# ajgupta93/d4pg-pytorch

Hardware: NVIDIA H100
Metric: learner grad-steps/sec (batch 256, 51 atoms) (higher is better)
Workload: dtype f32

## Files before the change

d4pg-pytorch_b200/csrc/learner.cu:

```cuda
#include "common.cuh"
#include "gemm_ffma.cuh"
#include "adam.cuh"
#include <string.h>
#include <stdlib.h>
#include <initializer_list>
#include <new>
#include <string>
#include <vector>

#include "internal.cuh"
#include "mlp_chain.cuh"
#include "mlp_tc_chain.cuh"

namespace d4pg {

struct Batch { float *s, *a, *s2; double* r; uint8_t* done; int32_t* idx; float* wts; uint8_t* hz; };

struct Workspace {
  Batch batch[2];
  float *h1[5], *h2[5], *h3[5], *out[5];
  float *m, *q_probs, *target_probs, *dlogits_q, *dlogits_pi, *loss_rows, *pi_rows;
  float *c_dz22, *c_dz2, *c_dz1, *p_dz22, *p_dz2, *a_dz3, *a_dz22, *a_dh2, *a_dz1;
  LearnerClock* clock;
  float* xchg;
  unsigned long long* pipe_epoch;
  double* sq_partials;
  int64_t total;
};

enum StepPlan { PLAN_LEVELS, PLAN_CHAIN, PLAN_TC_CHAIN };
constexpr int CHAIN_MAX_BATCH = 512;
static bool chain_pre_ok(const d4pg_learner_config_t& c) { return c.precision == 0 && c.act_dim <= 8; }
static bool chain_plan_fits(const d4pg_learner_config_t& c) {
  const int H = D4PG_HIDDEN, S = c.obs_dim, A = c.act_dim, N = c.n_atoms;
  ChainArgs f, b;
  chain_args_begin(f, c.batch, nullptr, c.precision);
  chain_add(f, 0, chain_fwd(nullptr, 0, nullptr, H, S, EPI_BIAS_RELU, nullptr, 0, 1));
  chain_add(f, 0, chain_fwd(nullptr, 0, nullptr, H, H, EPI_BIAS_RELU, nullptr, 0, 1));
  ChainSlot fc2 = chain_fwd(nullptr, 0, nullptr, H, H + A, EPI_BIAS_RELU, nullptr, 0, 1);
  if (chain_pre_ok(c)) chain_pre_layer(fc2, nullptr, 0, nullptr, nullptr, 0, A, H, EPI_BIAS_TANH, nullptr, 0, 0, H, false);
  else chain_add(f, 0, chain_fwd(nullptr, 0, nullptr, A, H, EPI_BIAS_TANH, nullptr, 0, 1));
  chain_add(f, 0, fc2);
  chain_add(f, 0, chain_fwd(nullptr, 0, nullptr, N, H, EPI_BIAS, nullptr, 0, 0));
  chain_args_begin(b, c.batch, nullptr, c.precision);
  chain_add(b, 0, chain_dx(nullptr, 0, H, N, EPI_RELU_MASK, nullptr, 0, nullptr, 0, 1));
  chain_add(b, 0, chain_dx(nullptr, 0, H, H, EPI_RELU_MASK, nullptr, 0, nullptr, 0, 1));
  ChainSlot fc3 = chain_dx(nullptr, 0, H, A, EPI_RELU_MASK, nullptr, 0, nullptr, 0, 1);
// ... 21 lines not shown
  auto take = [&](int64_t n) { float* p = base ? base + off : nullptr; off += align4(n); return p; };
  const int H = D4PG_HIDDEN, Sp = pitch4(S), Ap = pitch4(A), Np = pitch4(N);
  auto take_rows = [&](Batch& h) {
    h.s = take(int64_t(B) * Sp); h.a = take(int64_t(B) * Ap); h.s2 = take(int64_t(B) * Sp);
    h.r = reinterpret_cast<double*>(take(int64_t(B) * 2));
    h.done = reinterpret_cast<uint8_t*>(take((B + 3) / 4));
  };
  take_rows(w.batch[0]);
  for (int k = 0; k < 5; ++k) {
    if (k != 4) w.h1[k] = take(int64_t(B) * H);
    w.h2[k] = take(int64_t(B) * H); w.h3[k] = take(int64_t(B) * H);
  }
  w.out[0] = take(int64_t(B) * Ap); w.out[3] = take(int64_t(B) * Ap);
  w.out[1] = take(int64_t(B) * Np); w.out[2] = take(int64_t(B) * Np); w.out[4] = take(int64_t(B) * Np);
  w.m = take(int64_t(B) * Np); w.q_probs = take(int64_t(B) * Np); w.target_probs = take(int64_t(B) * Np);
  w.dlogits_q = take(int64_t(B) * Np); w.dlogits_pi = take(int64_t(B) * Np);
  w.loss_rows = take(B); w.pi_rows = take(B);
  w.c_dz22 = take(int64_t(B) * H); w.c_dz2 = take(int64_t(B) * H); w.c_dz1 = take(int64_t(B) * H);
  w.p_dz22 = take(int64_t(B) * H); w.p_dz2 = take(int64_t(B) * H);
  w.a_dz3 = take(int64_t(B) * Ap); w.a_dz22 = take(int64_t(B) * H); w.a_dh2 = take(int64_t(B) * H);
  w.a_dz1 = take(int64_t(B) * H);
  w.clock = reinterpret_cast<LearnerClock*>(take(sizeof(LearnerClock) / 4 + 4));
  w.xchg = plan != PLAN_LEVELS ? take(std::max(chain_xchg_floats(B), tcc_xchg_floats(B))) : nullptr;
  w.pipe_epoch = reinterpret_cast<unsigned long long*>(take(2 * int64_t((B + SAMPLE_ROWS - 1) / SAMPLE_ROWS)));
  if (prefetch) {
    take_rows(w.batch[1]);
    for (int k = 0; k < 2; ++k) { w.batch[k].idx = reinterpret_cast<int32_t*>(take(B)); w.batch[k].wts = take(B); }
  }
  if (clip) w.sq_partials = reinterpret_cast<double*>(take(2 * GRAD_NORM_CTAS * 2));
  if (tails)
    for (int k = 0; k < (prefetch ? 2 : 1); ++k) w.batch[k].hz = reinterpret_cast<uint8_t*>(take((B + 3) / 4));
  w.total = off;
  return w;
}
}

using namespace d4pg;

struct d4pg_learner {
  d4pg_learner_config_t cfg;
  d4pg_learner_buffers_t buf;
  d4pg_replay* replay;
  d4pg_comm* comm;
  StepPlan plan;
  Workspace ws;
  NetDims da, dc;
// ... 136 lines not shown
}
#define RUN(name, repeatable, call) \
  do { if (int rc_ = run_launch(x, name, repeatable, [&] { return (call); })) return rc_; } while (0)
static int run_level(Step& x, std::initializer_list<GemmProblem> problems) {
  GemmBatch g;
  gemm_batch_begin(g);
  for (const GemmProblem& p : problems) gemm_batch_add(g, p);
  RUN("gemm_launch", !gemm_batch_has_splitk(g), gemm_launch(g, x.c.precision, x.st));
  return D4PG_OK;
}

static int sample_batch(Step& x) {
  const d4pg_learner_config_t& c = x.c;
  RUN("learner_sample", false,
      learner_sample(x.L->replay, x.B, c.prioritized, c.sample_mode == 0 ? x.b.uniforms : nullptr,
                     (c.sample_mode == 0 && !c.prioritized) ? x.b.positions : nullptr,
                     c.philox_seed, x.w.clock, x.L->clock_params,
                     x.bt.idx, x.bt.wts, x.bt.s, x.bt.a, x.bt.r, x.bt.s2, x.bt.done, x.bt.hz, x.Sp, x.Ap, x.L->norm_affine,
                     x.L->norm_clip, x.pf ? x.par : -1, x.st));
  return D4PG_OK;
}

static void tcc_begin(const Step& x, TccArgs& a, int step_slot) {
  tcc_args_begin(a, x.B, reinterpret_cast<uint8_t*>(x.w.xchg), x.c.precision == 1 ? 3 : 1);
  a.step_slot = step_slot;
}
static int tcc_fwd_group(TccArgs& fa, int ci, int sl, const Step& x, Net net, int l, float* C, int ldc, int publish) {
  const Layer y = layer(x.L, net, l);
  return tcc_slot_group(fa, ci, sl, x.L->tcc_img[fwd_image(net, l)], y.epi, y.bias, nullptr, 0, C, ldc, publish);
}
static void tcc_build_actor_critic(TccArgs& fa, int ci, const Step& x, Net an, Net cn, const float* s, int ka, int kc,
                                   bool keep, bool actor_only = false) {
  const Workspace& w = x.w;
  const int H = D4PG_HIDDEN;
  int l, p1, p2 = -1;
  tcc_chain_x0(fa, ci, s, x.Sp, x.S);
  l = tcc_slot_begin(fa, ci); tcc_slot_src_x(fa, ci, l);
  p1 = tcc_fwd_group(fa, ci, l, x, an, 0, keep ? w.h1[ka] : nullptr, H, 1);
  if (!actor_only) p2 = tcc_fwd_group(fa, ci, l, x, cn, 0, nullptr, H, 1);
  l = tcc_slot_begin(fa, ci); tcc_slot_src_plane(fa, ci, l, p1, 8);
  p1 = tcc_fwd_group(fa, ci, l, x, an, 1, keep ? w.h2[ka] : nullptr, H, 1);
  l = tcc_slot_begin(fa, ci); tcc_slot_src_plane(fa, ci, l, p1, 8);
  p1 = tcc_fwd_group(fa, ci, l, x, an, 2, keep ? w.h3[ka] : nullptr, H, 1);
  l = tcc_slot_begin(fa, ci); tcc_slot_src_plane(fa, ci, l, p1, 8);
  const int pa = tcc_fwd_group(fa, ci, l, x, an, 3, w.out[ka], x.Ap, 1);
  if (actor_only) return;
  l = tcc_slot_begin(fa, ci); tcc_slot_src_plane(fa, ci, l, p2, 8); tcc_slot_src_plane(fa, ci, l, pa, 1);
// ... 551 lines not shown
    const size_t nb = size_t(cfg->batch);
    bool ok = cudaEventCreateWithFlags(&L->ev_in, cudaEventDisableTiming) == cudaSuccess &&
              cudaEventCreateWithFlags(&L->ev_out, cudaEventDisableTiming) == cudaSuccess &&
              cudaHostAlloc(reinterpret_cast<void**>(&L->host_losses), 4 * sizeof(float), cudaHostAllocDefault) == cudaSuccess;
    for (int i = 0; i < 2 && ok; ++i)
      ok = cudaEventCreateWithFlags(&L->ev_loss[i], cudaEventDisableTiming) == cudaSuccess &&
           cudaHostAlloc(reinterpret_cast<void**>(&L->loss_ring[i]), 4 * sizeof(float), cudaHostAllocDefault) == cudaSuccess;
    for (int i = 0; i < 4 && ok; ++i)
      ok = cudaEventCreateWithFlags(&L->ev_h2d[i], cudaEventDisableTiming) == cudaSuccess &&
           cudaHostAlloc(reinterpret_cast<void**>(&L->host_u[i]), nb * sizeof(double), cudaHostAllocMapped) == cudaSuccess &&
           cudaHostAlloc(reinterpret_cast<void**>(&L->host_pos[i]), nb * sizeof(int32_t), cudaHostAllocMapped) == cudaSuccess;
    if (!ok) { set_error("d4pg_learner_create: pinned staging allocation failed"); delete L; return D4PG_ECUDA; }
  }
  if (cudaStreamCreateWithFlags(&L->side, cudaStreamNonBlocking) != cudaSuccess ||
      cudaEventCreateWithFlags(&L->ev_fork, cudaEventDisableTiming) != cudaSuccess ||
      cudaEventCreateWithFlags(&L->ev_join, cudaEventDisableTiming) != cudaSuccess ||
      cudaEventCreateWithFlags(&L->ev_fork2, cudaEventDisableTiming) != cudaSuccess ||
      cudaEventCreateWithFlags(&L->ev_join2, cudaEventDisableTiming) != cudaSuccess) {
    set_error("d4pg_learner_create: stream/event creation failed"); delete L; return D4PG_ECUDA;
  }
  trace_set_side_stream(L->side);
  cudaError_t e = cudaMemset(L->ws.clock, 0, sizeof(LearnerClock));
  if (e == cudaSuccess) e = cudaMemset(L->ws.pipe_epoch, 0, sizeof(unsigned long long) * size_t(cdiv(cfg->batch, SAMPLE_ROWS)));
  if (e != cudaSuccess) { set_error("d4pg_learner_create: %s", cudaGetErrorString(e)); delete L; return D4PG_ECUDA; }
  *out = L;
  return D4PG_OK;
}

extern "C" int32_t d4pg_learner_destroy(d4pg_learner_t* L) {
  if (!L) return D4PG_OK;
  for (int i = 0; i < 4; ++i) if (L->graph_exec[i]) cudaGraphExecDestroy(L->graph_exec[i]);
  for (int i = 0; i < 2; ++i) if (L->multi_exec[i]) cudaGraphExecDestroy(L->multi_exec[i]);
  cudaEventDestroy(L->ev_fork); cudaEventDestroy(L->ev_join); cudaEventDestroy(L->ev_fork2); cudaEventDestroy(L->ev_join2);
  cudaStreamDestroy(L->side);
  if (L->tcc_images) cudaFree(L->tcc_images);
  if (L->gtab) cudaFree(L->gtab);
  if (L->ing) { cudaStreamSynchronize(L->ing); cudaStreamDestroy(L->ing); }
  if (L->ev_ing) cudaEventDestroy(L->ev_ing);
  if (L->ev_in) cudaEventDestroy(L->ev_in);
  if (L->ev_out) cudaEventDestroy(L->ev_out);
  if (L->host_losses) cudaFreeHost(L->host_losses);
  for (int i = 0; i < 2; ++i) {
    if (L->ev_loss[i]) cudaEventDestroy(L->ev_loss[i]);
    if (L->loss_ring[i]) cudaFreeHost(L->loss_ring[i]);
  }
  for (int i = 0; i < 4; ++i) {
// ... 251 lines not shown

extern "C" int32_t d4pg_learner_tensor(d4pg_learner_t* L, const char* name, void** ptr, int64_t* count, int32_t* ld) {
  D4PG_REQUIRE(L && name && ptr && count && ld, D4PG_EINVAL, "d4pg_learner_tensor: null argument");
  const Workspace& w = L->ws; const Batch& bt = w.batch[L->last_par];
  const int64_t B = L->cfg.batch;
  const int Sp = pitch4(L->cfg.obs_dim), Ap = pitch4(L->cfg.act_dim), Np = pitch4(L->cfg.n_atoms);
  struct E { const char* n; void* p; int64_t c; int ld; };
  const E table[] = {
      {"s", bt.s, B * Sp, Sp}, {"a", bt.a, B * Ap, Ap}, {"r", bt.r, B, 1}, {"s2", bt.s2, B * Sp, Sp}, {"done", bt.done, B, 1},
      {"h", bt.hz, bt.hz ? B : 0, 1},
      {"target_logits", w.out[1], B * Np, Np}, {"q_logits", w.out[2], B * Np, Np}, {"pi_logits", w.out[4], B * Np, Np},
      {"m", w.m, B * Np, Np}, {"q_probs", w.q_probs, B * Np, Np}, {"target_probs", w.target_probs, B * Np, Np},
      {"dlogits_q", w.dlogits_q, B * Np, Np}, {"dlogits_pi", w.dlogits_pi, B * Np, Np},
      {"actor_out", w.out[3], B * Ap, Ap}, {"actor_target_out", w.out[0], B * Ap, Ap},
      {"loss_rows", w.loss_rows, B, 1}, {"pi_rows", w.pi_rows, B, 1},
      {"h1_c", w.h1[2], B * 256, 256}, {"h2_c", w.h2[2], B * 256, 256}, {"h3_c", w.h3[2], B * 256, 256},
      {"h1_a", w.h1[3], B * 256, 256}, {"h2_a", w.h2[3], B * 256, 256}, {"h3_a", w.h3[3], B * 256, 256},
      {"h2_p", w.h2[4], B * 256, 256}, {"h3_p", w.h3[4], B * 256, 256},
      {"h1_at", w.h1[0], B * 256, 256}, {"h2_at", w.h2[0], B * 256, 256}, {"h3_at", w.h3[0], B * 256, 256},
      {"h1_ct", w.h1[1], B * 256, 256}, {"h2_ct", w.h2[1], B * 256, 256}, {"h3_ct", w.h3[1], B * 256, 256},
      {"p_dz22", w.p_dz22, B * 256, 256}, {"p_dz2", w.p_dz2, B * 256, 256},
      {"c_dz22", w.c_dz22, B * 256, 256}, {"c_dz2", w.c_dz2, B * 256, 256}, {"c_dz1", w.c_dz1, B * 256, 256},
      {"a_dz3", w.a_dz3, B * Ap, Ap}, {"a_dz22", w.a_dz22, B * 256, 256}, {"a_dh2", w.a_dh2, B * 256, 256},
      {"a_dz1", w.a_dz1, B * 256, 256}};
  for (const E& e : table)
    if (e.p && strcmp(e.n, name) == 0) { *ptr = e.p; *count = e.c; *ld = e.ld; return D4PG_OK; }
  set_error("d4pg_learner_tensor: unknown tensor '%s'", name);
  return D4PG_EINVAL;
}
```

d4pg-pytorch_b200/csrc/mlp_tc_chain.cu:

```cuda
#include "mlp_tc_chain.cuh"
#include "tc_common.cuh"
#include <stdlib.h>
#include <string.h>

namespace d4pg {

using namespace tc;

constexpr uint32_t TCC_OFF_A = 0;
constexpr uint32_t TCC_OFF_W = TCC_ABUFS * TCC_A_CHUNK;
constexpr uint32_t TCC_OFF_BAR = TCC_OFF_W + TCC_MAX_CHUNKS * TCC_W_CHUNK;
constexpr uint32_t TCC_SMEM = TCC_OFF_BAR + 256 + 1024;
static_assert(TCC_SMEM <= 227 * 1024, "the chain kernel's shared memory exceeds what a Hopper CTA may use");
constexpr int TCC_CONSUMERS = 256;
constexpr int TCC_TRACE_PER_SLOT = 12;

__device__ __forceinline__ void tcc_cluster_arrive() { asm volatile("barrier.cluster.arrive.release.aligned;" ::: "memory"); }
__device__ __forceinline__ void tcc_cluster_wait() { asm volatile("barrier.cluster.wait.acquire.aligned;" ::: "memory"); }
__device__ __forceinline__ unsigned tcc_ctarank() {
  unsigned r;
  asm volatile("mov.u32 %0, %%cluster_ctarank;" : "=r"(r));
  return r;
}
__device__ __forceinline__ unsigned long long tcc_gtime() {
// ... 10 lines not shown
  const long long t0 = clock64();
  bool recorded = false;
  while (!mbar_try_wait(bar, parity)) {
    const long long dt = clock64() - t0;
    if (dt > 4000000000ll && !recorded) {
      recorded = true;
      if (dbg) {
        if (atomicCAS(dbg, 0ull, 1ull) == 0ull) {
          dbg[1] = (unsigned long long)code | ((unsigned long long)parity << 24) | ((unsigned long long)blockIdx.x << 32);
          dbg[2] = aux;
        }
        const unsigned kind = code & 0xFFu;
        if (kind < 6 && atomicCAS(dbg + 4 + 2 * kind, 0ull, 1ull) == 0ull) {
          dbg[4 + 2 * kind] = (unsigned long long)code | ((unsigned long long)parity << 24) | ((unsigned long long)blockIdx.x << 32);
          dbg[5 + 2 * kind] = aux;
        }
        __threadfence_system();
      }
    }
    if (dt > 5000000000ll) __trap();
  }
}
#define TCC_CODE(kind, slot, rank) (unsigned(kind) | (unsigned(slot) << 8) | (unsigned(rank) << 16))
enum { WD_LOADER_DFULL = 2, WD_MMA_WFULL = 3, WD_MMA_FULL = 4 };

__device__ __forceinline__ float4 tcc_hi4(float4 v) { return make_float4(tf32_hi(v.x), tf32_hi(v.y), tf32_hi(v.z), tf32_hi(v.w)); }
__device__ __forceinline__ float4 tcc_lo4(float4 v, float4 h) {
  return make_float4(tf32_lo(v.x, h.x), tf32_lo(v.y, h.y), tf32_lo(v.z, h.z), tf32_lo(v.w, h.w));
}

__device__ __forceinline__ void tcc_convert_chunk(uint8_t* dst, const float* __restrict__ src, int ld, int k0, int ncols,
                                                  int m0, int B, int et) {
#pragma unroll
  for (int p = 0; p < 2; ++p) {
    const int e = et + p * 256, row = e >> 3, u = e & 7, k = k0 + (u << 2);
    float4 v = make_float4(0.f, 0.f, 0.f, 0.f);
    if (m0 + row < B && k < ncols) {
      v = __ldg(reinterpret_cast<const float4*>(src + size_t(m0 + row) * ld + k));
      if (k + 1 >= ncols) v.y = 0.f;
      if (k + 2 >= ncols) v.z = 0.f;
      if (k + 3 >= ncols) v.w = 0.f;
    }
    const float4 h = tcc_hi4(v);
    const uint32_t off = sw128_kmajor_off(row, u << 2);
    *reinterpret_cast<float4*>(dst + off) = h;
    *reinterpret_cast<float4*>(dst + TCC_A_HALF + off) = tcc_lo4(v, h);
  }
// ... 7 lines not shown
  uint32_t bytes = 0;
#pragma unroll
  for (int g = 0; g < TCC_MAX_GROUPS; ++g)
    if (tcc_group_active(S, g, n0)) bytes += gbytes;
  mbar_expect_tx(wfull, bytes);
#pragma unroll
  for (int g = 0; g < TCC_MAX_GROUPS; ++g)
    if (tcc_group_active(S, g, n0)) tcc_bulk_load(Wb + g * gbytes, S.g[g].wimg + size_t(rank) * gbytes, gbytes, wfull);
}

template <int PASSES>
__global__ void __cluster_dims__(TCC_CLUSTER, 1, 1) __launch_bounds__(TCC_THREADS, 1)
mlp_tc_chain_kernel(const __grid_constant__ TccArgs args) {
  static_assert(PASSES == 1 || PASSES == 3, "the chain kernel runs one TF32 pass or 3xTF32");
  extern __shared__ uint8_t tcc_smem_raw[];
  uint8_t* smem = reinterpret_cast<uint8_t*>((reinterpret_cast<uintptr_t>(tcc_smem_raw) + 1023) & ~uintptr_t(1023));
  uint8_t* Ab = smem + TCC_OFF_A;
  uint8_t* Xb = Ab + 8 * TCC_A_CHUNK;
  uint8_t* Wb = smem + TCC_OFF_W;
  uint64_t* bars = reinterpret_cast<uint64_t*>(smem + TCC_OFF_BAR);
  uint64_t* full = bars;
  uint64_t* wfull = bars + TCC_ABUFS;
  uint64_t* dfull = wfull + 1;

  const int tid = threadIdx.x, warp = tid >> 5, lane = tid & 31;
  const int rank = int(tcc_ctarank());
  const int cid = blockIdx.x / TCC_CLUSTER;
  const int chain = cid / args.row_blocks, rb = cid - chain * args.row_blocks;
  const int m0 = rb * TCC_ROWS, B = args.B;
  const TccChain& CH = args.chain[chain];
  const int ns = CH.nslots;
  const int n0 = rank * TCC_BN;
  uint8_t* planes = args.xchg + (size_t(chain) * args.row_blocks + rb) * (size_t(TCC_PLANES) * TCC_PLANE_BYTES);
  const int npre = CH.pre ? (CH.precols + TCC_KC - 1) / TCC_KC : 0;
  unsigned long long* tr0 = (args.trace && int(blockIdx.x) == args.trace_cta) ? args.trace : nullptr;
  if (args.wait_epoch) {
    if (tid < args.wait_n) {
      const unsigned long long target = (unsigned long long)(*reinterpret_cast<const volatile long long*>(args.wait_clock) + 1);
      unsigned long long v;
      do { asm volatile("ld.acquire.gpu.global.u64 %0, [%1];" : "=l"(v) : "l"(args.wait_epoch + tid) : "memory"); } while (v < target);
    }
    __syncthreads();
  }
  step_stamp(args.step_trace, args.step_slot);

  if (tid == TCC_CONSUMERS) {
    for (int i = 0; i < TCC_ABUFS + 2; ++i) mbar_init(&bars[i], 1);
    mbar_fence_init();
  }
  if (tid < TCC_CONSUMERS) {
    if (CH.x0) tcc_convert_chunk(Xb, CH.x0, CH.x0ld, 0, CH.x0cols, m0, B, tid);
    for (int p = 0; p < npre; ++p) tcc_convert_chunk(Ab + p * TCC_A_CHUNK, CH.pre, CH.preld, p * TCC_KC, CH.precols, m0, B, tid);
    fence_proxy_async();
  }
  __syncthreads();

  if (tid == TCC_CONSUMERS)
    for (int p = 0; p < npre; ++p) mbar_arrive(&full[p]);
  uint32_t fph = 0;
  int nact = 0;
  if (tid == TCC_CONSUMERS && tcc_slot_active(CH.slot[0], n0)) tcc_issue_weights(CH.slot[0], rank, n0, Wb, wfull);

  for (int l = 0; l < ns; ++l) {
    const TccSlot& S = CH.slot[l];
    const bool active = tcc_slot_active(S, n0);
    unsigned long long* tr = tr0 ? tr0 + TCC_TRACE_PER_SLOT * l : nullptr;
    bool arrived = false;

    if (tid >= TCC_CONSUMERS) {
      if (lane == 0) {
        if (tr) tr[0] = tcc_gtime();
        if (active && S.nloads > 0) {
          asm volatile("fence.proxy.async.global;" ::: "memory");
          for (int i = 0; i < S.nloads; ++i) {
            const TccLoad L = S.ld[i];
            const uint32_t bytes = uint32_t(L.count) * TCC_A_CHUNK;
            mbar_expect_tx(&full[L.buf0], bytes);
            tcc_bulk_load(Ab + L.buf0 * TCC_A_CHUNK, planes + size_t(L.plane) * TCC_PLANE_BYTES + size_t(L.chunk0) * TCC_A_CHUNK,
                          bytes, &full[L.buf0]);
          }
        }
        if (tr) tr[1] = tcc_gtime();
        if (l + 1 < ns && tcc_slot_active(CH.slot[l + 1], n0)) {
          if (active) tcc_wait(dfull, nact & 1, args.watchdog, TCC_CODE(WD_LOADER_DFULL, l, rank), nact);
          tcc_issue_weights(CH.slot[l + 1], rank, n0, Wb, wfull);
        }
      }
      __syncwarp();
    } else {
      const int g = warp >> 2, wq = warp & 3;
      const bool mine = tcc_group_active(S, g, n0);
      const int rl = 16 * wq + (lane >> 2);
      const int cl = 2 * (lane & 3);
      if (active) {
        const TccGroup& G = S.g[g];
        constexpr int N1 = PASSES == 3 ? 32 : 16;
        float d1[N1], d2[PASSES == 3 ? 16 : 1];
#pragma unroll
        for (int i = 0; i < N1; ++i) d1[i] = 0.f;
        if constexpr (PASSES == 3) {
#pragma unroll
          for (int i = 0; i < 16; ++i) d2[i] = 0.f;
        }
        float eop[2][8];
        const int npad = mine ? (G.N + 3) & ~3 : 0;
        const bool fwd = G.epi == EPI_BIAS || G.epi == EPI_BIAS_RELU || G.epi == EPI_BIAS_TANH;
        const bool msk = G.epi == EPI_RELU_MASK || G.epi == EPI_TANH_MASK;
// ... 30 lines not shown
            const uint32_t w = w_base + uint32_t(c) * TCC_W_CHUNK;
            wg_fence();
#pragma unroll
            for (int ks = 0; ks < 4; ++ks) {
              const uint64_t bd = wg_desc(w + 32 * ks);
              if constexpr (PASSES == 3) {
                wg_mma_n64(d1, wg_desc(a_hi + 32 * ks), bd);
                wg_mma_n32(d2, wg_desc(a_lo + 32 * ks), bd);
              } else {
                wg_mma_n32(d1, wg_desc(a_hi + 32 * ks), bd);
              }
            }
            wg_commit();
          }
          wg_wait<0>();
          wg_fence_regs(d1);
          if constexpr (PASSES == 3) wg_fence_regs(d2);
          if (tr && tid == 0) tr[4] = tcc_gtime();
        }
        for (int c = 0; c < nch; ++c)
          if ((wait_mask >> c) & 1u) fph ^= 1u << (c + boff);
        asm volatile("bar.sync 1, %0;" ::"n"(TCC_CONSUMERS) : "memory");
        if (tid == 0) mbar_arrive(dfull);
        if (tr && tid == 0) tr[5] = tcc_gtime();
        if (S.xsrc) {
          tcc_convert_chunk(Xb, S.xsrc, S.xld, 0, S.xcols, m0, B, tid);
          fence_proxy_async();
        }
        if (mine) {
          const int epi = G.epi;
          float x[16];
          if constexpr (PASSES == 3) {
#pragma unroll
            for (int i = 0; i < 16; ++i) x[i] = (d1[i + 16] + d2[i]) + d1[i];
          } else {
#pragma unroll
            for (int i = 0; i < 16; ++i) x[i] = d1[i];
          }
#pragma unroll
          for (int i = 0; i < 16; ++i) {
            const float e = eop[(i >> 1) & 1][2 * (i >> 2) + (i & 1)];
            if (epi == EPI_BIAS || epi == EPI_BIAS_RELU || epi == EPI_BIAS_TANH) x[i] += e;
            else if (epi == EPI_RELU_MASK) x[i] = (e > 0.f) ? x[i] : 0.f;
            else if (epi == EPI_TANH_MASK) x[i] *= (1.f - e * e);
          }
          if (epi == EPI_BIAS_RELU) {
// ... 9 lines not shown
            const int gi = m0 + rl + 8 * ((i >> 1) & 1), gj = n0 + 8 * (i >> 2) + cl + (i & 1);
            x[i] = (gi < B && gj < G.N) ? x[i] : 0.f;
          }
          if (tr && tid == 0) tr[6] = tcc_gtime();
          if (G.pub >= 0) {
            uint8_t* stg = Ab + (2 + g) * TCC_A_CHUNK;
#pragma unroll
            for (int i = 0; i < 16; i += 2) {
              const int r = rl + 8 * ((i >> 1) & 1), k = 8 * (i >> 2) + cl;
              const float2 v = make_float2(x[i], x[i + 1]);
              const float2 h = make_float2(tf32_hi(v.x), tf32_hi(v.y));
              const uint32_t off = sw128_kmajor_off(r, k);
              *reinterpret_cast<float2*>(stg + off) = h;
              *reinterpret_cast<float2*>(stg + TCC_A_HALF + off) = make_float2(tf32_lo(v.x, h.x), tf32_lo(v.y, h.y));
            }
            fence_proxy_async();
            asm volatile("bar.sync %0, 128;" ::"r"(2 + g) : "memory");
            if ((tid & 127) == 0) {
              uint8_t* img = planes + size_t(G.pub) * TCC_PLANE_BYTES + size_t(rank) * TCC_A_CHUNK;
              asm volatile("cp.async.bulk.global.shared::cta.bulk_group [%0], [%1], %2;"
                           ::"l"(img), "r"(smem_u32(stg)), "r"(TCC_A_CHUNK) : "memory");
              asm volatile("cp.async.bulk.commit_group;" ::: "memory");
              asm volatile("cp.async.bulk.wait_group 0;" ::: "memory");
            }
          }
          if (tr && tid == 0) tr[8] = tcc_gtime();
          if (l + 1 < ns) { tcc_cluster_arrive(); arrived = true; }
          if (G.C) {
#pragma unroll
            for (int i = 0; i < 16; i += 2) {
              const int gi = m0 + rl + 8 * ((i >> 1) & 1), gj = n0 + 8 * (i >> 2) + cl;
              if (gi < B && gj < npad) *reinterpret_cast<float2*>(G.C + size_t(gi) * G.ldc + gj) = make_float2(x[i], x[i + 1]);
            }
          }
        }
      } else if (S.xsrc) {
        tcc_convert_chunk(Xb, S.xsrc, S.xld, 0, S.xcols, m0, B, tid);
        fence_proxy_async();
      }
      if (tr && tid == 0) tr[9] = tcc_gtime();
    }
    if (active) ++nact;
    if (l + 1 < ns) {
      if (!arrived) tcc_cluster_arrive();
      tcc_cluster_wait();
      if (tr && tid == 0) tr[10] = tcc_gtime();
    }
  }
  step_stamp(args.step_trace, args.step_slot + 16);
}

__global__ void __launch_bounds__(256) tcc_pack_kernel(const __grid_constant__ TccPackArgs args) {
  int ui = 0;
#pragma unroll 1
  for (int i = 1; i < args.n; ++i)
    if (int(blockIdx.x) >= args.use[i].block_begin) ui = i;
  const TccPackUse& U = args.use[ui];
  const int blk = blockIdx.x - U.block_begin;
  const int slice = blk / U.nchunks, chunk = blk - slice * U.nchunks;
  uint8_t* dst = args.dst + U.dst_off + size_t(blk) * TCC_W_CHUNK;
  const int tid = threadIdx.x;
  float4 v = make_float4(0.f, 0.f, 0.f, 0.f);
  int j, u;
  if (U.mode == GEMM_FWD) {
    j = tid >> 3; u = tid & 7;
    const int n = slice * TCC_BN + j, k = chunk * TCC_KC + 4 * u;
    if (n < U.N && k < U.K) {
      v = __ldg(reinterpret_cast<const float4*>(U.W + size_t(n) * U.ldw + k));
      if (k + 1 >= U.K) v.y = 0.f;
      if (k + 2 >= U.K) v.z = 0.f;
      if (k + 3 >= U.K) v.w = 0.f;
// ... 41 lines not shown
void tcc_pack_begin(TccPackArgs& p, uint8_t* dst) { p.n = 0; p.total_blocks = 0; p.dst = dst; }
int tcc_pack_add(TccPackArgs& p, const float* W, int ldw, int mode, int N, int K) {
  if (p.n >= TCC_MAX_USES) return -1;
  TccPackUse& u = p.use[p.n];
  u.W = W; u.ldw = ldw; u.mode = mode; u.N = N; u.K = K;
  u.nslices = cdiv(N, TCC_BN); u.nchunks = cdiv(K, TCC_KC);
  u.block_begin = p.total_blocks;
  u.dst_off = (long long)(p.total_blocks) * TCC_W_CHUNK;
  p.total_blocks += u.nslices * u.nchunks;
  return p.n++;
}
long long tcc_pack_bytes(const TccPackArgs& p) { return (long long)(p.total_blocks) * TCC_W_CHUNK; }
void tcc_pack_set_base(TccPackArgs& p, uint8_t* dst, long long first_byte) { p.dst = dst + first_byte; }
int launch_tcc_pack(const TccPackArgs& p, cudaStream_t st) {
  D4PG_REQUIRE(p.n > 0 && p.dst, D4PG_EINVAL, "launch_tcc_pack: nothing to pack");
  tcc_pack_kernel<<<p.total_blocks, 256, 0, st>>>(p);
  D4PG_LAUNCH_OK();
  return D4PG_OK;
}

int64_t tcc_xchg_floats(int B) {
  return int64_t(TCC_MAX_CHAINS) * cdiv(B, TCC_ROWS) * TCC_PLANES * (TCC_PLANE_BYTES / 4);
}
void tcc_args_begin(TccArgs& a, int B, uint8_t* xchg, int passes) {
  memset(&a, 0, sizeof(a));
  a.B = B; a.row_blocks = cdiv(B, TCC_ROWS); a.xchg = xchg; a.passes = passes;
}
void tcc_chain_x0(TccArgs& a, int c, const float* src, int ld, int cols) {
  a.chain[c].x0 = src; a.chain[c].x0ld = ld; a.chain[c].x0cols = cols;
}
void tcc_chain_pre(TccArgs& a, int c, const float* src, int ld, int cols) {
  a.chain[c].pre = src; a.chain[c].preld = ld; a.chain[c].precols = cols;
}
int tcc_slot_begin(TccArgs& a, int c) {
  if (c >= a.nchains) a.nchains = c + 1;
  TccChain& ch = a.chain[c];
  const int l = ch.nslots++;
  if (l < TCC_MAX_SLOTS) { ch.slot[l] = TccSlot{}; ch.slot[l].g[0].pub = ch.slot[l].g[1].pub = -1; }
  return l;
}
static void tcc_push_chunk(TccSlot& s, int kind, int plane, int chunk) {
  if (s.nchunks < TCC_MAX_CHUNKS) s.ch[s.nchunks] = TccChunk{short(kind), short(plane), short(chunk), 0};
  ++s.nchunks;
}
void tcc_slot_src_x(TccArgs& a, int c, int slot) { tcc_push_chunk(a.chain[c].slot[slot], TCC_SRC_X, 0, 0); }
void tcc_slot_src_pre(TccArgs& a, int c, int slot) {
  const int n = cdiv(a.chain[c].precols, TCC_KC);
  for (int i = 0; i < n; ++i) tcc_push_chunk(a.chain[c].slot[slot], TCC_SRC_PRE, 0, i);
}
void tcc_slot_src_plane(TccArgs& a, int c, int slot, int plane, int nchunks) {
  for (int i = 0; i < nchunks; ++i) tcc_push_chunk(a.chain[c].slot[slot], TCC_SRC_IMG, plane, i);
}
void tcc_slot_reconvert_x(TccArgs& a, int c, int slot, const float* src, int ld, int cols) {
  TccSlot& s = a.chain[c].slot[slot];
  s.xsrc = src; s.xld = ld; s.xcols = cols;
}
int tcc_slot_group(TccArgs& a, int c, int slot, const TccImage& img, int epi, const float* bias,
                   const float* aux, int ldaux, float* C, int ldc, int publish) {
  TccChain& ch = a.chain[c];
  TccSlot& s = ch.slot[slot];
  const int gi = s.ngroups++;
  if (gi >= TCC_MAX_GROUPS) return -1;
  TccGroup& g = s.g[gi];
  g.wimg = img.ptr; g.bias = bias; g.aux = aux; g.ldaux = ldaux; g.C = C; g.ldc = ldc;
  g.N = img.N; g.epi = epi; g.kchunks = img.kchunks;
  g.pub = publish ? ch.nplanes++ : -1;
  return g.pub;
}

int launch_mlp_tc_chain(TccArgs& a, cudaStream_t st) {
  D4PG_REQUIRE(a.nchains > 0 && a.nchains <= TCC_MAX_CHAINS, D4PG_EINVAL, "launch_mlp_tc_chain: %d chains", a.nchains);
  D4PG_REQUIRE(a.passes == 1 || a.passes == 3, D4PG_EINVAL, "launch_mlp_tc_chain: passes %d", a.passes);
  constexpr int gmax = 2;
  for (int c = 0; c < a.nchains; ++c) {
    TccChain& ch = a.chain[c];
    bool x_clobbered = false;
    D4PG_REQUIRE(ch.nslots > 0 && ch.nslots <= TCC_MAX_SLOTS, D4PG_EINVAL, "launch_mlp_tc_chain: chain %d has %d slots", c, ch.nslots);
    D4PG_REQUIRE(ch.nplanes <= TCC_PLANES, D4PG_ENOTSUP, "launch_mlp_tc_chain: chain %d publishes %d planes", c, ch.nplanes);
    D4PG_REQUIRE(!ch.x0 || (ch.x0cols <= TCC_KC && ch.x0ld % 4 == 0 && ch.x0ld >= ch.x0cols), D4PG_ENOTSUP, "launch_mlp_tc_chain: bad X source");
    D4PG_REQUIRE(!ch.pre || (ch.precols <= 8 * TCC_KC && ch.preld % 4 == 0 && ch.preld >= ch.precols), D4PG_ENOTSUP,
                 "launch_mlp_tc_chain: bad first-slot source");
    int planes_seen = 0;
    for (int l = 0; l < ch.nslots; ++l) {
      TccSlot& s = ch.slot[l];
      D4PG_REQUIRE(s.ngroups >= 1 && s.ngroups <= TCC_MAX_GROUPS, D4PG_EINVAL, "launch_mlp_tc_chain: slot %d has %d groups", l, s.ngroups);
      D4PG_REQUIRE(s.nchunks >= 1 && s.nchunks <= TCC_MAX_CHUNKS && s.ngroups * s.nchunks <= TCC_MAX_CHUNKS, D4PG_ENOTSUP,
                   "launch_mlp_tc_chain: slot %d: %d groups x %d chunks exceed the weight buffer", l, s.ngroups, s.nchunks);
      int nring = 0;
      bool uses_x = false;
      for (int i = 0; i < s.nchunks; ++i) uses_x = uses_x || s.ch[i].kind == TCC_SRC_X;
      s.nloads = 0;
      for (int i = 0; i < s.nchunks; ++i) {
        TccChunk& k = s.ch[i];
        if (k.kind == TCC_SRC_IMG) D4PG_REQUIRE(k.plane >= 0 && k.plane < planes_seen && k.chunk < TCC_CLUSTER, D4PG_EINVAL,
                                                 "launch_mlp_tc_chain: slot %d reads plane %d before it is published", l, k.plane);
        if (k.kind == TCC_SRC_PRE) D4PG_REQUIRE(l == 0 && ch.pre && k.chunk == nring && nring < 8, D4PG_EINVAL, "launch_mlp_tc_chain: pre chunks belong to slot 0, in order");
        if (k.kind == TCC_SRC_X) {
          D4PG_REQUIRE(ch.x0 != nullptr && !x_clobbered, D4PG_EINVAL, "launch_mlp_tc_chain: slot %d reads X but the chain has none (or it was overwritten)", l);
          k.buf = 8;
          continue;
        }
        if (nring < 8) k.buf = short(nring);
        else {
          D4PG_REQUIRE(nring == 8 && !uses_x && k.kind == TCC_SRC_IMG, D4PG_ENOTSUP, "launch_mlp_tc_chain: slot %d needs more than 9 A buffers", l);
          k.buf = 8; x_clobbered = true;
        }
        ++nring;
        if (k.kind == TCC_SRC_IMG) {
          TccLoad* cur = s.nloads ? &s.ld[s.nloads - 1] : nullptr;
          if (cur && cur->plane == k.plane && cur->chunk0 + cur->count == k.chunk && cur->buf0 + cur->count == k.buf && cur->count < gmax) ++cur->count;
          else s.ld[s.nloads++] = TccLoad{k.plane, k.chunk, k.buf, 1};
        }
      }
      s.boff = s.ch[0].buf;
      s.wait_mask = 0;
      for (int i = 0; i < s.nchunks; ++i) {
        D4PG_REQUIRE(s.ch[i].buf == s.boff + i, D4PG_ENOTSUP, "launch_mlp_tc_chain: slot %d: chunk %d is not in A buffer %d", l, i, s.boff + i);
        if (s.ch[i].kind == TCC_SRC_PRE) s.wait_mask |= 1u << i;
      }
      for (int i = 0; i < s.nloads; ++i) s.wait_mask |= 1u << (s.ld[i].buf0 - s.boff);
      for (int g = 0; g < s.ngroups; ++g) {
        const TccGroup& G = s.g[g];
        D4PG_REQUIRE(G.N > 0 && G.N <= TCC_CLUSTER * TCC_BN && G.wimg, D4PG_ENOTSUP, "launch_mlp_tc_chain: group width %d", G.N);
        D4PG_REQUIRE(G.kchunks == s.nchunks, D4PG_EINVAL, "launch_mlp_tc_chain: chain %d slot %d: A operand has %d chunks, the weight image %d", c, l, s.nchunks, G.kchunks);
        D4PG_REQUIRE(!G.C || (G.ldc % 4 == 0 && G.ldc >= ((G.N + 3) & ~3) && (reinterpret_cast<uintptr_t>(G.C) & 15) == 0), D4PG_EINVAL,
                     "launch_mlp_tc_chain: output pitch");
        const bool fwd = G.epi == EPI_BIAS || G.epi == EPI_BIAS_RELU || G.epi == EPI_BIAS_TANH;
        const bool msk = G.epi == EPI_RELU_MASK || G.epi == EPI_TANH_MASK;
        D4PG_REQUIRE(!fwd || (G.bias && (reinterpret_cast<uintptr_t>(G.bias) & 15) == 0), D4PG_EINVAL, "launch_mlp_tc_chain: bias");
        D4PG_REQUIRE(!msk || (G.aux && G.ldaux % 4 == 0 && (reinterpret_cast<uintptr_t>(G.aux) & 15) == 0), D4PG_EINVAL, "launch_mlp_tc_chain: mask operand");
        if (G.pub >= 0) ++planes_seen;
      }
      if (l == 0 && ch.pre) D4PG_REQUIRE(s.g[0].N > (TCC_CLUSTER - 1) * TCC_BN, D4PG_ENOTSUP, "launch_mlp_tc_chain: the first slot must span the cluster");
    }
  }
  void (*kern)(TccArgs) = a.passes == 3 ? mlp_tc_chain_kernel<3> : mlp_tc_chain_kernel<1>;
  static bool attr_set[2] = {false, false};
  const int ai = a.passes == 3 ? 1 : 0;
  if (!attr_set[ai]) {
    D4PG_CUDA_OK(cudaFuncSetAttribute(kern, cudaFuncAttributeMaxDynamicSharedMemorySize, int(TCC_SMEM)));
    D4PG_CUDA_OK(cudaFuncSetAttribute(kern, cudaFuncAttributePreferredSharedMemoryCarveout, int(cudaSharedmemCarveoutMaxShared)));
    attr_set[ai] = true;
  }
  a.watchdog = tcc_watchdog_device();
  unsigned long long* dbg = debug_trace_buffer();
  a.trace = dbg ? dbg + (a.step_slot == 5 ? 384 : 256) : nullptr;
  a.step_trace = dbg ? dbg + STEP_TRACE_BASE : nullptr;
  { const char* e = getenv("D4PG_TRACE_CTA"); a.trace_cta = e ? atoi(e) : 0; if (a.trace_cta >= a.nchains * a.row_blocks * TCC_CLUSTER) a.trace_cta = 0; }
  cudaLaunchConfig_t cfg{};
  cfg.gridDim = dim3(a.nchains * a.row_blocks * TCC_CLUSTER); cfg.blockDim = dim3(TCC_THREADS);
  cfg.dynamicSmemBytes = TCC_SMEM; cfg.stream = st;
  cfg.attrs = nullptr; cfg.numAttrs = 0;
  D4PG_CUDA_OK(cudaLaunchKernelEx(&cfg, kern, a));
  return D4PG_OK;
// ... 4 lines not shown
```

d4pg-pytorch_b200/csrc/mlp_tc_chain.cuh:

```cuda
#pragma once
#include "gemm_ffma.cuh"

namespace d4pg {

constexpr int TCC_ROWS = 64;
constexpr int TCC_CLUSTER = 8;
constexpr int TCC_BN = 32;
constexpr int TCC_KC = 32;
constexpr int TCC_ABUFS = 9;
constexpr int TCC_MAX_SLOTS = 8, TCC_MAX_CHAINS = 3, TCC_MAX_GROUPS = 2, TCC_MAX_CHUNKS = 9, TCC_PLANES = 8;
constexpr uint32_t TCC_A_HALF = TCC_ROWS * 128, TCC_A_CHUNK = 2 * TCC_A_HALF;
constexpr uint32_t TCC_W_HALF = TCC_BN * 128, TCC_W_CHUNK = 2 * TCC_W_HALF;
constexpr uint32_t TCC_PLANE_BYTES = TCC_CLUSTER * TCC_A_CHUNK;
constexpr int TCC_THREADS = 288;

enum { TCC_SRC_IMG = 0, TCC_SRC_X = 1, TCC_SRC_PRE = 2 };

struct TccGroup {
  const uint8_t* wimg;
  const float* bias;
  const float* aux; int ldaux;
  float* C; int ldc;
  int N, epi, kchunks;
  int pub;
};
struct TccChunk { short kind, plane, chunk, buf; };
struct TccLoad { short plane, chunk0, buf0, count; };
struct TccSlot {
  TccGroup g[TCC_MAX_GROUPS];
  TccChunk ch[TCC_MAX_CHUNKS];
  TccLoad ld[TCC_MAX_CHUNKS];
  int ngroups, nchunks, nloads;
  int boff; unsigned wait_mask;
  const float* xsrc; int xld, xcols;
};
struct TccChain {
  TccSlot slot[TCC_MAX_SLOTS];
  int nslots, nplanes;
  const float* x0; int x0ld, x0cols;
  const float* pre; int preld, precols;
};
struct TccArgs {
  TccChain chain[TCC_MAX_CHAINS];
  int nchains, B, row_blocks;
  int passes;
  const unsigned long long* wait_epoch; const long long* wait_clock; int wait_n;
  uint8_t* xchg;
  unsigned long long* trace; int trace_cta;
  unsigned long long* step_trace; int step_slot;
  unsigned long long* watchdog;
};

struct TccPackUse {
  const float* W; int ldw, mode, N, K;
  int nslices, nchunks, block_begin;
  long long dst_off;
};
constexpr int TCC_MAX_USES = 32;
struct TccPackArgs {
  TccPackUse use[TCC_MAX_USES];
  int n, total_blocks;
  uint8_t* dst;
};
void tcc_pack_begin(TccPackArgs& p, uint8_t* dst);
int tcc_pack_add(TccPackArgs& p, const float* W, int ldw, int mode, int N, int K);
void tcc_pack_set_base(TccPackArgs& p, uint8_t* dst, long long first_byte);
long long tcc_pack_bytes(const TccPackArgs& p);
struct TccImage { const uint8_t* ptr; int N, kchunks; };
static inline TccImage tcc_image(const TccPackArgs& p, int use) { return TccImage{p.dst + p.use[use].dst_off, p.use[use].N, p.use[use].nchunks}; }
int launch_tcc_pack(const TccPackArgs& p, cudaStream_t st);

int64_t tcc_xchg_floats(int B);
void tcc_args_begin(TccArgs& a, int B, uint8_t* xchg, int passes);
void tcc_chain_x0(TccArgs& a, int c, const float* src, int ld, int cols);
void tcc_chain_pre(TccArgs& a, int c, const float* src, int ld, int cols);
int tcc_slot_begin(TccArgs& a, int c);
void tcc_slot_src_x(TccArgs& a, int c, int slot);
void tcc_slot_src_pre(TccArgs& a, int c, int slot);
void tcc_slot_src_plane(TccArgs& a, int c, int slot, int plane, int nchunks);
void tcc_slot_reconvert_x(TccArgs& a, int c, int slot, const float* src, int ld, int cols);
int tcc_slot_group(TccArgs& a, int c, int slot, const TccImage& img, int epi, const float* bias,
                   const float* aux, int ldaux, float* C, int ldc, int publish);
int launch_mlp_tc_chain(TccArgs& a, cudaStream_t st);
unsigned long long* tcc_watchdog_device();

}
```

Measured before the change: 7302.

## Replace per-slot cluster barriers with per-chunk epoch flags in TC chain kernel

Removes the cluster-wide arrive/wait between every layer slot of the tensor-core MLP chain. Each CTA now publishes its plane chunk with a release store of a launch epoch to a global flag. Loaders poll those flags with acquire loads and issue bulk loads for chunks as soon as they are ready. An 'afree' mbarrier keeps A buffers from being refilled while still in use. This should let CTAs proceed at their own pace and overlap layers, at the cost of global flag polling, more watchdog logic and extra validation constraints.

```diff
diff --git a/d4pg-pytorch_b200/csrc/learner.cu b/d4pg-pytorch_b200/csrc/learner.cu
--- a/d4pg-pytorch_b200/csrc/learner.cu
+++ b/d4pg-pytorch_b200/csrc/learner.cu
@@ -23,6 +23,7 @@
   float *c_dz22, *c_dz2, *c_dz1, *p_dz22, *p_dz2, *a_dz3, *a_dz22, *a_dh2, *a_dz1;
   LearnerClock* clock;
   float* xchg;
+  unsigned long long* tcc_sync;
   unsigned long long* pipe_epoch;
   double* sq_partials;
   int64_t total;
@@ -90,6 +91,7 @@
   w.a_dz1 = take(int64_t(B) * H);
   w.clock = reinterpret_cast<LearnerClock*>(take(sizeof(LearnerClock) / 4 + 4));
   w.xchg = plan != PLAN_LEVELS ? take(std::max(chain_xchg_floats(B), tcc_xchg_floats(B))) : nullptr;
+  w.tcc_sync = plan == PLAN_TC_CHAIN ? reinterpret_cast<unsigned long long*>(take(tcc_sync_floats(B))) : nullptr;
   w.pipe_epoch = reinterpret_cast<unsigned long long*>(take(2 * int64_t((B + SAMPLE_ROWS - 1) / SAMPLE_ROWS)));
   if (prefetch) {
     take_rows(w.batch[1]);
@@ -272,7 +274,7 @@
 }
 
 static void tcc_begin(const Step& x, TccArgs& a, int step_slot) {
-  tcc_args_begin(a, x.B, reinterpret_cast<uint8_t*>(x.w.xchg), x.c.precision == 1 ? 3 : 1);
+  tcc_args_begin(a, x.B, reinterpret_cast<uint8_t*>(x.w.xchg), x.w.tcc_sync, x.c.precision == 1 ? 3 : 1);
   a.step_slot = step_slot;
 }
 static int tcc_fwd_group(TccArgs& fa, int ci, int sl, const Step& x, Net net, int l, float* C, int ldc, int publish) {
@@ -870,6 +872,7 @@
   trace_set_side_stream(L->side);
   cudaError_t e = cudaMemset(L->ws.clock, 0, sizeof(LearnerClock));
   if (e == cudaSuccess) e = cudaMemset(L->ws.pipe_epoch, 0, sizeof(unsigned long long) * size_t(cdiv(cfg->batch, SAMPLE_ROWS)));
+  if (e == cudaSuccess && L->ws.tcc_sync) e = cudaMemset(L->ws.tcc_sync, 0, sizeof(float) * size_t(tcc_sync_floats(cfg->batch)));
   if (e != cudaSuccess) { set_error("d4pg_learner_create: %s", cudaGetErrorString(e)); delete L; return D4PG_ECUDA; }
   *out = L;
   return D4PG_OK;
@@ -1167,7 +1170,8 @@
       {"p_dz22", w.p_dz22, B * 256, 256}, {"p_dz2", w.p_dz2, B * 256, 256},
       {"c_dz22", w.c_dz22, B * 256, 256}, {"c_dz2", w.c_dz2, B * 256, 256}, {"c_dz1", w.c_dz1, B * 256, 256},
       {"a_dz3", w.a_dz3, B * Ap, Ap}, {"a_dz22", w.a_dz22, B * 256, 256}, {"a_dh2", w.a_dh2, B * 256, 256},
-      {"a_dz1", w.a_dz1, B * 256, 256}};
+      {"a_dz1", w.a_dz1, B * 256, 256},
+      {"tcc_sync", w.tcc_sync, int64_t(TCC_MAX_CHAINS) * cdiv(L->cfg.batch, TCC_ROWS) * TCC_SYNC_WORDS, TCC_SYNC_WORDS}};
   for (const E& e : table)
     if (e.p && strcmp(e.n, name) == 0) { *ptr = e.p; *count = e.c; *ld = e.ld; return D4PG_OK; }
   set_error("d4pg_learner_tensor: unknown tensor '%s'", name);
diff --git a/d4pg-pytorch_b200/csrc/mlp_tc_chain.cu b/d4pg-pytorch_b200/csrc/mlp_tc_chain.cu
--- a/d4pg-pytorch_b200/csrc/mlp_tc_chain.cu
+++ b/d4pg-pytorch_b200/csrc/mlp_tc_chain.cu
@@ -56,7 +56,30 @@
   }
 }
 #define TCC_CODE(kind, slot, rank) (unsigned(kind) | (unsigned(slot) << 8) | (unsigned(rank) << 16))
-enum { WD_LOADER_DFULL = 2, WD_MMA_WFULL = 3, WD_MMA_FULL = 4 };
+enum { WD_LOADER_AFREE = 1, WD_LOADER_DFULL = 2, WD_MMA_WFULL = 3, WD_MMA_FULL = 4, WD_LOADER_FLAG = 5 };
+
+__device__ __forceinline__ unsigned long long tcc_ld_acquire(const unsigned long long* p) {
+  unsigned long long v;
+  asm volatile("ld.acquire.gpu.global.u64 %0, [%1];" : "=l"(v) : "l"(p) : "memory");
+  return v;
+}
+__device__ __forceinline__ void tcc_flag_watchdog(long long dt, bool& recorded, unsigned long long* dbg, unsigned code, unsigned aux) {
+  if (dt > 4000000000ll && !recorded) {
+    recorded = true;
+    if (dbg) {
+      if (atomicCAS(dbg, 0ull, 1ull) == 0ull) {
+        dbg[1] = (unsigned long long)code | ((unsigned long long)blockIdx.x << 32);
+        dbg[2] = aux;
+      }
+      if (atomicCAS(dbg + 4 + 2 * WD_LOADER_FLAG, 0ull, 1ull) == 0ull) {
+        dbg[4 + 2 * WD_LOADER_FLAG] = (unsigned long long)code | ((unsigned long long)blockIdx.x << 32);
+        dbg[5 + 2 * WD_LOADER_FLAG] = aux;
+      }
+      __threadfence_system();
+    }
+  }
+  if (dt > 5000000000ll) __trap();
+}
 
 __device__ __forceinline__ float4 tcc_hi4(float4 v) { return make_float4(tf32_hi(v.x), tf32_hi(v.y), tf32_hi(v.z), tf32_hi(v.w)); }
 __device__ __forceinline__ float4 tcc_lo4(float4 v, float4 h) {
@@ -110,6 +133,7 @@
   uint64_t* full = bars;
   uint64_t* wfull = bars + TCC_ABUFS;
   uint64_t* dfull = wfull + 1;
+  uint64_t* afree = dfull + 1;
 
   const int tid = threadIdx.x, warp = tid >> 5, lane = tid & 31;
   const int rank = int(tcc_ctarank());
@@ -120,6 +144,9 @@
   const int ns = CH.nslots;
   const int n0 = rank * TCC_BN;
   uint8_t* planes = args.xchg + (size_t(chain) * args.row_blocks + rb) * (size_t(TCC_PLANES) * TCC_PLANE_BYTES);
+  unsigned long long* sync = args.sync + size_t(cid) * TCC_SYNC_WORDS;
+  unsigned long long* flags = sync + TCC_SYNC_FLAGS;
+  const unsigned long long epoch = *reinterpret_cast<const volatile unsigned long long*>(sync) + 1;
   const int npre = CH.pre ? (CH.precols + TCC_KC - 1) / TCC_KC : 0;
   unsigned long long* tr0 = (args.trace && int(blockIdx.x) == args.trace_cta) ? args.trace : nullptr;
   if (args.wait_epoch) {
@@ -134,6 +161,7 @@
 
   if (tid == TCC_CONSUMERS) {
     for (int i = 0; i < TCC_ABUFS + 2; ++i) mbar_init(&bars[i], 1);
+    mbar_init(afree, 2);
     mbar_fence_init();
   }
   if (tid < TCC_CONSUMERS) {
@@ -147,30 +175,52 @@
     for (int p = 0; p < npre; ++p) mbar_arrive(&full[p]);
   uint32_t fph = 0;
   int nact = 0;
+  int dseen = 0, fseen = 0;
   if (tid == TCC_CONSUMERS && tcc_slot_active(CH.slot[0], n0)) tcc_issue_weights(CH.slot[0], rank, n0, Wb, wfull);
 
   for (int l = 0; l < ns; ++l) {
     const TccSlot& S = CH.slot[l];
     const bool active = tcc_slot_active(S, n0);
     unsigned long long* tr = tr0 ? tr0 + TCC_TRACE_PER_SLOT * l : nullptr;
-    bool arrived = false;
 
     if (tid >= TCC_CONSUMERS) {
+      if (tr && lane == 0) tr[0] = tcc_gtime();
+      if (active && S.nloads > 0) {
+        if (lane == 0)
+          for (; fseen < nact; ++fseen) tcc_wait(afree, fseen & 1, args.watchdog, TCC_CODE(WD_LOADER_AFREE, l, rank), fseen);
+        const unsigned long long* f = nullptr;
+        if (lane < S.nchunks && S.ch[lane].kind == TCC_SRC_IMG) f = flags + S.ch[lane].plane * TCC_CLUSTER + S.ch[lane].chunk;
+        uint32_t ready = 0;
+        int i = 0;
+        const long long t0 = clock64();
+        bool recorded = false;
+        while (i < S.nloads) {
+          const bool ok = !f || ((ready >> lane) & 1u) || tcc_ld_acquire(f) >= epoch;
+          ready = __ballot_sync(0xFFFFFFFFu, ok);
+          __syncwarp();
+          if (lane == 0) {
+            bool fenced = false;
+            for (; i < S.nloads; ++i) {
+              const TccLoad L = S.ld[i];
+              const uint32_t m = ((1u << L.count) - 1u) << (L.buf0 - S.boff);
+              if ((ready & m) != m) break;
+              if (!fenced) { asm volatile("fence.proxy.async.global;" ::: "memory"); fenced = true; }
+              const uint32_t bytes = uint32_t(L.count) * TCC_A_CHUNK;
+              mbar_expect_tx(&full[L.buf0], bytes);
+              tcc_bulk_load(Ab + L.buf0 * TCC_A_CHUNK, planes + size_t(L.plane) * TCC_PLANE_BYTES + size_t(L.chunk0) * TCC_A_CHUNK,
+                            bytes, &full[L.buf0]);
+            }
+          }
+          i = __shfl_sync(0xFFFFFFFFu, i, 0);
+          if (!ok) tcc_flag_watchdog(clock64() - t0, recorded, args.watchdog, TCC_CODE(WD_LOADER_FLAG, l, rank), unsigned(lane));
+        }
+        if (tr && lane == 0) tr[10] = tcc_gtime();
+      }
       if (lane == 0) {
-        if (tr) tr[0] = tcc_gtime();
-        if (active && S.nloads > 0) {
-          asm volatile("fence.proxy.async.global;" ::: "memory");
-          for (int i = 0; i < S.nloads; ++i) {
-            const TccLoad L = S.ld[i];
-            const uint32_t bytes = uint32_t(L.count) * TCC_A_CHUNK;
-            mbar_expect_tx(&full[L.buf0], bytes);
-            tcc_bulk_load(Ab + L.buf0 * TCC_A_CHUNK, planes + size_t(L.plane) * TCC_PLANE_BYTES + size_t(L.chunk0) * TCC_A_CHUNK,
-                          bytes, &full[L.buf0]);
-          }
-        }
         if (tr) tr[1] = tcc_gtime();
         if (l + 1 < ns && tcc_slot_active(CH.slot[l + 1], n0)) {
-          if (active) tcc_wait(dfull, nact & 1, args.watchdog, TCC_CODE(WD_LOADER_DFULL, l, rank), nact);
+          for (const int n = nact + (active ? 1 : 0); dseen < n; ++dseen)
+            tcc_wait(dfull, dseen & 1, args.watchdog, TCC_CODE(WD_LOADER_DFULL, l, rank), dseen);
           tcc_issue_weights(CH.slot[l + 1], rank, n0, Wb, wfull);
         }
       }
@@ -247,6 +297,8 @@
           if ((wait_mask >> c) & 1u) fph ^= 1u << (c + boff);
         asm volatile("bar.sync 1, %0;" ::"n"(TCC_CONSUMERS) : "memory");
         if (tid == 0) mbar_arrive(dfull);
+        const bool stages = mine && G.pub >= 0;
+        if (!stages && (tid & 127) == 0) mbar_arrive(afree);
         if (tr && tid == 0) tr[5] = tcc_gtime();
         if (S.xsrc) {
           tcc_convert_chunk(Xb, S.xsrc, S.xld, 0, S.xcols, m0, B, tid);
@@ -302,10 +354,13 @@
                            ::"l"(img), "r"(smem_u32(stg)), "r"(TCC_A_CHUNK) : "memory");
               asm volatile("cp.async.bulk.commit_group;" ::: "memory");
               asm volatile("cp.async.bulk.wait_group 0;" ::: "memory");
+              mbar_arrive(afree);
+              asm volatile("fence.proxy.async.global;" ::: "memory");
+              asm volatile("st.release.gpu.global.u64 [%0], %1;"
+                           ::"l"(flags + G.pub * TCC_CLUSTER + rank), "l"(epoch) : "memory");
             }
           }
           if (tr && tid == 0) tr[8] = tcc_gtime();
-          if (l + 1 < ns) { tcc_cluster_arrive(); arrived = true; }
           if (G.C) {
 #pragma unroll
             for (int i = 0; i < 16; i += 2) {
@@ -321,12 +376,10 @@
       if (tr && tid == 0) tr[9] = tcc_gtime();
     }
     if (active) ++nact;
-    if (l + 1 < ns) {
-      if (!arrived) tcc_cluster_arrive();
-      tcc_cluster_wait();
-      if (tr && tid == 0) tr[10] = tcc_gtime();
-    }
-  }
+  }
+  tcc_cluster_arrive();
+  tcc_cluster_wait();
+  if (rank == 0 && tid == 0) *reinterpret_cast<volatile unsigned long long*>(sync) = epoch;
   step_stamp(args.step_trace, args.step_slot + 16);
 }
 
@@ -414,9 +467,10 @@
 int64_t tcc_xchg_floats(int B) {
   return int64_t(TCC_MAX_CHAINS) * cdiv(B, TCC_ROWS) * TCC_PLANES * (TCC_PLANE_BYTES / 4);
 }
-void tcc_args_begin(TccArgs& a, int B, uint8_t* xchg, int passes) {
+int64_t tcc_sync_floats(int B) { return int64_t(TCC_MAX_CHAINS) * cdiv(B, TCC_ROWS) * TCC_SYNC_WORDS * 2; }
+void tcc_args_begin(TccArgs& a, int B, uint8_t* xchg, unsigned long long* sync, int passes) {
   memset(&a, 0, sizeof(a));
-  a.B = B; a.row_blocks = cdiv(B, TCC_ROWS); a.xchg = xchg; a.passes = passes;
+  a.B = B; a.row_blocks = cdiv(B, TCC_ROWS); a.xchg = xchg; a.sync = sync; a.passes = passes;
 }
 void tcc_chain_x0(TccArgs& a, int c, const float* src, int ld, int cols) {
   a.chain[c].x0 = src; a.chain[c].x0ld = ld; a.chain[c].x0cols = cols;
@@ -463,18 +517,22 @@
 int launch_mlp_tc_chain(TccArgs& a, cudaStream_t st) {
   D4PG_REQUIRE(a.nchains > 0 && a.nchains <= TCC_MAX_CHAINS, D4PG_EINVAL, "launch_mlp_tc_chain: %d chains", a.nchains);
   D4PG_REQUIRE(a.passes == 1 || a.passes == 3, D4PG_EINVAL, "launch_mlp_tc_chain: passes %d", a.passes);
+  D4PG_REQUIRE(a.xchg && a.sync, D4PG_EINVAL, "launch_mlp_tc_chain: no exchange planes or slot flags");
   constexpr int gmax = 2;
   for (int c = 0; c < a.nchains; ++c) {
     TccChain& ch = a.chain[c];
-    bool x_clobbered = false;
+    bool x_clobbered = false, x_reconverted = false;
     D4PG_REQUIRE(ch.nslots > 0 && ch.nslots <= TCC_MAX_SLOTS, D4PG_EINVAL, "launch_mlp_tc_chain: chain %d has %d slots", c, ch.nslots);
-    D4PG_REQUIRE(ch.nplanes <= TCC_PLANES, D4PG_ENOTSUP, "launch_mlp_tc_chain: chain %d publishes %d planes", c, ch.nplanes);
+    D4PG_REQUIRE(ch.nplanes <= TCC_PLANES, D4PG_ENOTSUP,
+                 "launch_mlp_tc_chain: chain %d publishes %d planes; every publish of a launch needs a plane of its own "
+                 "(none is rewritten within a launch) and there are %d", c, ch.nplanes, TCC_PLANES);
     D4PG_REQUIRE(!ch.x0 || (ch.x0cols <= TCC_KC && ch.x0ld % 4 == 0 && ch.x0ld >= ch.x0cols), D4PG_ENOTSUP, "launch_mlp_tc_chain: bad X source");
     D4PG_REQUIRE(!ch.pre || (ch.precols <= 8 * TCC_KC && ch.preld % 4 == 0 && ch.preld >= ch.precols), D4PG_ENOTSUP,
                  "launch_mlp_tc_chain: bad first-slot source");
-    int planes_seen = 0;
+    int planes_seen = 0, plane_n[TCC_PLANES] = {};
     for (int l = 0; l < ch.nslots; ++l) {
       TccSlot& s = ch.slot[l];
+      x_reconverted = x_reconverted || s.xsrc != nullptr;
       D4PG_REQUIRE(s.ngroups >= 1 && s.ngroups <= TCC_MAX_GROUPS, D4PG_EINVAL, "launch_mlp_tc_chain: slot %d has %d groups", l, s.ngroups);
       D4PG_REQUIRE(s.nchunks >= 1 && s.nchunks <= TCC_MAX_CHUNKS && s.ngroups * s.nchunks <= TCC_MAX_CHUNKS, D4PG_ENOTSUP,
                    "launch_mlp_tc_chain: slot %d: %d groups x %d chunks exceed the weight buffer", l, s.ngroups, s.nchunks);
@@ -484,8 +542,12 @@
       s.nloads = 0;
       for (int i = 0; i < s.nchunks; ++i) {
         TccChunk& k = s.ch[i];
-        if (k.kind == TCC_SRC_IMG) D4PG_REQUIRE(k.plane >= 0 && k.plane < planes_seen && k.chunk < TCC_CLUSTER, D4PG_EINVAL,
-                                                 "launch_mlp_tc_chain: slot %d reads plane %d before it is published", l, k.plane);
+        if (k.kind == TCC_SRC_IMG) {
+          D4PG_REQUIRE(k.plane >= 0 && k.plane < planes_seen && k.chunk < TCC_CLUSTER, D4PG_EINVAL,
+                       "launch_mlp_tc_chain: slot %d reads plane %d before it is published", l, k.plane);
+          D4PG_REQUIRE(k.chunk * TCC_BN < plane_n[k.plane], D4PG_EINVAL,
+                       "launch_mlp_tc_chain: slot %d reads chunk %d of plane %d, which is %d wide", l, k.chunk, k.plane, plane_n[k.plane]);
+        }
         if (k.kind == TCC_SRC_PRE) D4PG_REQUIRE(l == 0 && ch.pre && k.chunk == nring && nring < 8, D4PG_EINVAL, "launch_mlp_tc_chain: pre chunks belong to slot 0, in order");
         if (k.kind == TCC_SRC_X) {
           D4PG_REQUIRE(ch.x0 != nullptr && !x_clobbered, D4PG_EINVAL, "launch_mlp_tc_chain: slot %d reads X but the chain has none (or it was overwritten)", l);
@@ -495,6 +557,7 @@
         if (nring < 8) k.buf = short(nring);
         else {
           D4PG_REQUIRE(nring == 8 && !uses_x && k.kind == TCC_SRC_IMG, D4PG_ENOTSUP, "launch_mlp_tc_chain: slot %d needs more than 9 A buffers", l);
+          D4PG_REQUIRE(!x_reconverted, D4PG_ENOTSUP, "launch_mlp_tc_chain: slot %d reuses the X buffer of a chain that re-converts X", l);
           k.buf = 8; x_clobbered = true;
         }
         ++nring;
@@ -511,6 +574,7 @@
         if (s.ch[i].kind == TCC_SRC_PRE) s.wait_mask |= 1u << i;
       }
       for (int i = 0; i < s.nloads; ++i) s.wait_mask |= 1u << (s.ld[i].buf0 - s.boff);
+      D4PG_REQUIRE(l == 0 || s.nloads > 0, D4PG_ENOTSUP, "launch_mlp_tc_chain: slot %d loads no plane chunk", l);
       for (int g = 0; g < s.ngroups; ++g) {
         const TccGroup& G = s.g[g];
         D4PG_REQUIRE(G.N > 0 && G.N <= TCC_CLUSTER * TCC_BN && G.wimg, D4PG_ENOTSUP, "launch_mlp_tc_chain: group width %d", G.N);
@@ -521,7 +585,7 @@
         const bool msk = G.epi == EPI_RELU_MASK || G.epi == EPI_TANH_MASK;
         D4PG_REQUIRE(!fwd || (G.bias && (reinterpret_cast<uintptr_t>(G.bias) & 15) == 0), D4PG_EINVAL, "launch_mlp_tc_chain: bias");
         D4PG_REQUIRE(!msk || (G.aux && G.ldaux % 4 == 0 && (reinterpret_cast<uintptr_t>(G.aux) & 15) == 0), D4PG_EINVAL, "launch_mlp_tc_chain: mask operand");
-        if (G.pub >= 0) ++planes_seen;
+        if (G.pub >= 0) { plane_n[G.pub] = G.N; ++planes_seen; }
       }
       if (l == 0 && ch.pre) D4PG_REQUIRE(s.g[0].N > (TCC_CLUSTER - 1) * TCC_BN, D4PG_ENOTSUP, "launch_mlp_tc_chain: the first slot must span the cluster");
     }
diff --git a/d4pg-pytorch_b200/csrc/mlp_tc_chain.cuh b/d4pg-pytorch_b200/csrc/mlp_tc_chain.cuh
--- a/d4pg-pytorch_b200/csrc/mlp_tc_chain.cuh
+++ b/d4pg-pytorch_b200/csrc/mlp_tc_chain.cuh
@@ -13,6 +13,7 @@
 constexpr uint32_t TCC_W_HALF = TCC_BN * 128, TCC_W_CHUNK = 2 * TCC_W_HALF;
 constexpr uint32_t TCC_PLANE_BYTES = TCC_CLUSTER * TCC_A_CHUNK;
 constexpr int TCC_THREADS = 288;
+constexpr int TCC_SYNC_FLAGS = 8, TCC_SYNC_WORDS = TCC_SYNC_FLAGS + TCC_PLANES * TCC_CLUSTER;
 
 enum { TCC_SRC_IMG = 0, TCC_SRC_X = 1, TCC_SRC_PRE = 2 };
 
@@ -46,6 +47,7 @@
   int passes;
   const unsigned long long* wait_epoch; const long long* wait_clock; int wait_n;
   uint8_t* xchg;
+  unsigned long long* sync;
   unsigned long long* trace; int trace_cta;
   unsigned long long* step_trace; int step_slot;
   unsigned long long* watchdog;
@@ -71,7 +73,8 @@
 int launch_tcc_pack(const TccPackArgs& p, cudaStream_t st);
 
 int64_t tcc_xchg_floats(int B);
-void tcc_args_begin(TccArgs& a, int B, uint8_t* xchg, int passes);
+int64_t tcc_sync_floats(int B);
+void tcc_args_begin(TccArgs& a, int B, uint8_t* xchg, unsigned long long* sync, int passes);
 void tcc_chain_x0(TccArgs& a, int c, const float* src, int ld, int cols);
 void tcc_chain_pre(TccArgs& a, int c, const float* src, int ld, int cols);
 int tcc_slot_begin(TccArgs& a, int c);
```

After: 6209, median of 6. 15.0% lower.
